# pbluc/avrecode-ms

Measured on AMD Instinct MI355X. Metric: H.264 bytes/s recompressed (CABAC re-encode of recorded bin streams, bit-exact vs CPU), higher is better.
Workload: dtype u32

## Files before the change

avrecode-ms_amd/csrc/avr_api.cpp:

```cpp
#include <hip/hip_runtime.h>

#include <algorithm>
#include <cstdarg>
#include <cstdio>
#include <cstdlib>
#include <cstring>
#include <mutex>
#include <new>
#include <numeric>
#include <string>
#include <thread>
#include <vector>

#include "avr_internal.h"
#include "avr_synth.h"
#include "avr_tables.h"

namespace {

thread_local char g_err[512] = "";

int fail(int code, const char *fmt, ...) {
    va_list ap;
    va_start(ap, fmt);
// ... 125 lines not shown
    avr_chunk_plan plan{};

    bool verify = false;
    bool verified = false;
    hipEvent_t vev[3] = {};
    float verify_ms = 0;
    DevBuf<uint32_t> d_first_bad;
    PinBuf<uint32_t> h_first_bad;
};

template <class T>
static int stage_h2d(avr_batch *b, T *dst, const T *src, size_t n) {
    const size_t bytes = n * sizeof(T), at = (b->plan_used + 63) & ~size_t(63);
    if (at + bytes > b->h_plan.cap) return fail(AVR_ERR_NOMEM, "plan staging area too small (%zu + %zu > %zu)", at, bytes, b->h_plan.cap);
    memcpy(b->h_plan.p + at, src, bytes);
    b->plan_used = at + bytes;
    AVR_HIP(hipMemcpyAsync(dst, b->h_plan.p + at, bytes, hipMemcpyHostToDevice, b->stream));
    return AVR_OK;
}
namespace avr {
const Env &env() {
    static const Env e = [] {
        Env v{0, false, false};
        if (const char *p = getenv("AVR_K1_PATH")) v.k1_path = strcmp(p, "chunked") == 0 ? 2 : strcmp(p, "serial") == 0 ? 1 : 0;
        v.no_dense = getenv("AVR_NO_DENSE") != nullptr;
        v.no_hint = getenv("AVR_BATCH_NO_HINT") != nullptr;
        return v;
    }();
    return e;
}
#ifdef AVR_TEST_HOOKS
TestHooks &test_hooks() { static TestHooks h{}; return h; }
#endif
}

extern "C" {

#ifdef AVR_TEST_HOOKS
int avr_test_hook_set(const char *name, uint32_t value) {
    avr::TestHooks &h = avr::test_hooks();
    if (!name) return fail(AVR_ERR_INVALID, "null hook name");
    if (!strcmp(name, "k1p_force_retry_every")) h.k1p_force_retry_every = value;
    else if (!strcmp(name, "census_stride")) h.census_stride = value;
    else if (!strcmp(name, "chain_lanes")) h.chain_lanes = value;
    else if (!strcmp(name, "k1_form_ref")) h.k1_form_ref = value;
    else if (!strcmp(name, "k1_emit_lds")) h.k1_emit_lds = value;
    else if (!strcmp(name, "k1_path")) h.k1_path = value;
    else if (!strcmp(name, "no_dense")) h.no_dense = value;
    else if (!strcmp(name, "no_hint")) h.no_hint = value;
    else if (!strcmp(name, "k2p_seg_len")) h.k2p_seg_len = value;
    else if (!strcmp(name, "local_waves")) h.local_waves = value;
    else if (!strcmp(name, "k2p_wave")) h.k2p_wave = value;
    else if (!strcmp(name, "k1p_keep_retry")) h.k1p_keep_retry = value;
    else if (!strcmp(name, "k1_waves")) h.k1_waves = value;
    else if (!strcmp(name, "k1_fwd")) h.k1_fwd = value;
    else if (!strcmp(name, "k1_words8")) h.k1_words8 = value;
    else if (!strcmp(name, "chain_nsegs")) h.chain_nsegs = value;
    else if (!strcmp(name, "chain_whole")) h.chain_whole = value;
    else if (!strcmp(name, "chain_segments")) h.chain_segments = value;
    else if (!strcmp(name, "chain_force_redo")) h.chain_force_redo = value;
    else if (!strcmp(name, "verify_flip")) h.verify_flip = value;
    else if (!strcmp(name, "reset")) h = avr::TestHooks{};
    else return fail(AVR_ERR_INVALID, "unknown test hook %s", name);
    return AVR_OK;
}
#endif

const char *avr_last_error(void) { return g_err; }
const char *avr_version(void) { return "avrecode-ms_amd 0.1 (gfx950)"; }

int avr_device_count(void) {
    int n = 0;
    if (hipGetDeviceCount(&n) != hipSuccess) return 0;
    return n;
}

const uint8_t *avr_cabac_lps_range_table(void) { return kTables.lps_range; }
const uint8_t *avr_cabac_mlps_state_table(void) { return kTables.mlps_state; }


avr_batch *avr_batch_create(int device, size_t max_slices, size_t max_bins) {
    if (max_slices == 0 || max_slices > 0x7fffffffu) { fail(AVR_ERR_INVALID, "max_slices out of range"); return nullptr; }
    if (select_device(device) != AVR_OK) return nullptr;
    avr_batch *b = new (std::nothrow) avr_batch;
    if (!b) { fail(AVR_ERR_NOMEM, "out of host memory"); return nullptr; }
    b->device = device;
    b->max_slices = max_slices;
    b->max_bins = max_bins;
    bool ok = hipStreamCreateWithFlags(&b->stream, hipStreamNonBlocking) == hipSuccess;
    for (int i = 0; ok && i < 5; i++) ok = hipEventCreate(&b->ev[i]) == hipSuccess;
    ok = ok && b->h_recs.reserve(max_bins + 16 * max_slices) == AVR_OK;
    if (!ok) {
        if (!g_err[0]) fail(AVR_ERR_HIP, "stream/event creation failed");
        avr_batch_destroy(b);
        return nullptr;
    }
    b->rec_off.reserve(max_slices + 1);
    b->n_bins.reserve(max_slices);
    b->rec_off.push_back(0);
    return b;
}

void avr_batch_destroy(avr_batch *b) {
    if (!b) return;
    (void)hipSetDevice(b->device);
    if (b->stream) (void)hipStreamSynchronize(b->stream);
// ... 1217 lines not shown
```

avrecode-ms_amd/csrc/avr_internal.h:

```cpp
#pragma once
#include <hip/hip_runtime.h>
#include <stdint.h>

#include <list>
#include <mutex>

#include "../../include/avrecode_ms_amd.h"
#include "avr_layout.h"

#define AVR_NOP_CABAC2  (AVR_NOP_CABAC | (AVR_NOP_CABAC << 16))
#define AVR_SLICE_RETRY_SERIAL 100
#define AVR_SLICE_RETRY_CENSUS 101
#define AVR_SLICE_DONE         102

namespace avr {

struct Env { int k1_path; bool no_dense, no_hint; };
const Env &env();
struct TestHooks {
    uint32_t k1p_force_retry_every;
    uint32_t census_stride;
    uint32_t chain_lanes;
    uint32_t k1_form_ref;
    uint32_t k1_emit_lds;
    uint32_t k1_path, no_dense, no_hint;
    uint32_t chain_segments;
    uint32_t chain_whole;
    uint32_t chain_force_redo;
    uint32_t k2p_seg_len;
    uint32_t local_waves;
    uint32_t chain_nsegs;
    uint32_t k1_fwd;
    uint32_t k1_words8;
    uint32_t k1_waves;
    uint32_t k2p_wave;
    uint32_t verify_flip;
    uint32_t k1p_keep_retry;
};
#ifdef AVR_TEST_HOOKS
TestHooks &test_hooks();
#else
inline const TestHooks &test_hooks() { static const TestHooks none{}; return none; }
#endif
inline int k1_path() { return test_hooks().k1_path ? int(test_hooks().k1_path) : env().k1_path; }
inline bool no_dense() { return test_hooks().no_dense || env().no_dense; }
inline bool no_hint() { return test_hooks().no_hint || env().no_hint; }

struct DenseHint { uint32_t rows; uint32_t *host_count; uint32_t *host_retry; uint32_t sharing = 0; };

template <class T>
class StreamPool {
    struct Slot { int dev; hipStream_t s; T x; };
    std::list<Slot> slots_;
    std::mutex mu_;
public:
    template <class Make>
    hipError_t get(hipStream_t s, T **out, Make make) {
        int dev = 0;
        hipError_t e = hipGetDevice(&dev);
        if (e != hipSuccess) return e;
        std::lock_guard<std::mutex> lock(mu_);
        for (Slot &x : slots_)
            if (x.dev == dev && x.s == s) { *out = &x.x; return hipSuccess; }
        T fresh{};
        if ((e = make(fresh)) != hipSuccess) return e;
        slots_.push_back(Slot{dev, s, fresh});
        *out = &slots_.back().x;
        return hipSuccess;
    }
    template <class Destroy>
    void forget(hipStream_t s, Destroy destroy) {
        std::lock_guard<std::mutex> lock(mu_);
        for (auto it = slots_.begin(); it != slots_.end();)
            if (it->s == s) { destroy(it->x); it = slots_.erase(it); } else ++it;
    }
};

void forget_stream(hipStream_t s);
void forget_part_streams(hipStream_t s);

hipError_t launch_cabac_encode(bool tiled, hipStream_t s, const void *recs, const uint64_t *off,
                               const uint32_t *n_bins, const uint32_t *order, uint32_t n_slices,
                               const uint8_t *init_states, uint32_t n_states, uint8_t *out,
                               const uint64_t *out_off, uint32_t *out_len, int32_t *status,
                               uint8_t *final_states, int32_t want_status = AVR_SLICE_OK, bool dense = true,
                               const DenseHint *hint = nullptr);
hipError_t launch_densemap(hipStream_t s, const uint32_t *used, uint16_t *table, uint16_t *index, uint32_t *n_dense);
hipError_t launch_range_encode(bool tiled, hipStream_t s, const void *recs, const uint64_t *off,
                               const uint32_t *n_bins, const uint32_t *order, uint32_t n_slices,
                               uint8_t *out, const uint64_t *out_off, uint32_t *out_len,
// ... 60 lines not shown
```

avrecode-ms_amd/csrc/avr_k1p.h:

```cpp
#pragma once
#include <stdint.h>

#if defined(__HIPCC__)
#define AVR_HD __host__ __device__ inline
#else
#define AVR_HD inline
#endif

namespace avr {
namespace k1p {

#if defined(__HIP_DEVICE_COMPILE__)
#define AVR_PIN2(a, b) asm volatile("" : "+v"(a), "+v"(b))
#else
#define AVR_PIN2(a, b) ((void)0)
#endif

constexpr uint32_t kChunk = 1024;
constexpr uint32_t kNone = 0xffffffffu;
constexpr uint32_t kMaxStretch = 16 * kChunk;
constexpr uint32_t kCodeBypass = 252;
constexpr uint32_t kCodePad = 252;

struct alignas(16) U4 { uint32_t x, y, z, w; };
// ... 196 lines not shown
            const U4 v = *reinterpret_cast<const U4 *>(res + i);
            const uint32_t w[4] = {v.x, v.y, v.z, v.w};
#if defined(__HIP_DEVICE_COMPILE__)
#pragma unroll 1
#endif
            for (uint32_t k = 0; k < 4; k++) {
                CodeEntry e[4];
                code_entries4(codes, w[k], e);
                for (uint32_t b = 0; b < 4; b++)
                    for (uint32_t q = 0; q < 4; q++) T[q] += step_range(e[b], &R[q]);
            }
            i += 16;
        }
        code_by_code(n);
    }
    uint32_t Rm = R[0], Tm = 0, end = i;
    if (!closed && i < n) {
        const uint32_t interior_end = limit < n ? limit : n;
        if (i < interior_end) {
            for_codes_all(res, i, interior_end, [&](uint32_t c) { Tm += step_range(codes[c], &Rm); },
                          [&](uint32_t d) {
                              CodeEntry e[4];
                              code_entries4(codes, d, e);
                              Tm += step_range(e[0], &Rm); Tm += step_range(e[1], &Rm);
                              Tm += step_range(e[2], &Rm); Tm += step_range(e[3], &Rm);
                          });
            i = interior_end;
        }
        end = n;
        for_codes(res, i, n, [&](uint32_t idx, uint32_t c) {
            const bool closing = idx >= limit && code_is_boundary(c);
            if (closing) o->exit_q = uint8_t(((Rm >> 6) & 3) * 0x55u);
            Tm += step_range(codes[c], &Rm);
            if (closing) { end = idx + 1; return true; }
            if (idx - lo > max_stretch) { o->too_long = 1; end = idx + 1; return true; }
            return false;
        });
        R[0] = R[1] = R[2] = R[3] = Rm;
    }
    o->end = end;
    for (uint32_t q = 0; q < 4; q++) { o->t_exit[q] = T[q] + Tm; o->r_exit[q] = uint16_t(R[q]); }
}


struct Entry {
    uint32_t t_start;
    uint32_t q;
};

struct SliceTotals {
    uint32_t t_total;
    uint32_t r_final;
    uint32_t bad;
    uint32_t pad;
};

AVR_HD void b2_chain(const Stretch *st, uint32_t n_chunks, Entry *en, SliceTotals *tot) {
    uint32_t T = 0, q = 0, r = 510, bad = 0;
    for (uint32_t c = 0; c < n_chunks; c++) {
        if (st[c].first == kNone) continue;
        en[c].t_start = T;
        en[c].q = q;
        T += st[c].t_exit[q];
        r = st[c].r_exit[q];
        bad |= st[c].too_long;
        q = (st[c].exit_q >> (2 * q)) & 3;
    }
    tot->t_total = T;
    tot->r_final = r;
    tot->bad = bad;
    tot->pad = 0;
}

AVR_HD uint32_t ref_digits(uint32_t t) { return t <= 21 ? 0 : (t - 21 + 15) / 16; }


template <class A, class = void> struct adder_is_staged { static constexpr bool value = false; };
template <class A> struct adder_is_staged<A, decltype(void(A::kStaged))> { static constexpr bool value = A::kStaged; };
template <class Src, class Adder>
AVR_HD void c_stretch_in(const Src &src, const Stretch &st, const Entry &en, uint32_t chunk,
                         const CodeEntryC *codes, Adder &S) {
    uint32_t R, from;
    if (chunk == 0) { R = 510; from = 0; }
    else { uint32_t sh; R = post_lps_range(codes[src.byte(st.first)].row, en.q, &sh); from = st.first + 1; }
    const uint32_t phase = en.t_start & 15, g0 = en.t_start >> 4;
    uint64_t L2 = 0;
    int sp = int(phase) - 7;
    uint32_t j = 0;
    constexpr bool staged = adder_is_staged<Adder>::value;
    if constexpr (staged) S.begin(g0);
    auto bin_e = [&](const CodeEntryC &e) {
        uint32_t v;
        const uint32_t sh = step_range_c(e, &R, &v);
        L2 = (L2 + v) << sh;
        sp += int(sh);
    };
    auto bin = [&](uint32_t c) { bin_e(codes[c]); };
    auto put = [&](uint32_t d) {
        if constexpr (staged) S.push(g0 + j, d);
        else if (j < 2) S.add(g0 + j, d);
        else S.store(g0 + j, d);
        j++;
    };
    auto digits = [&]() {
        while (sp >= 15) {
            const uint32_t d = uint32_t(L2 >> (sp + 1));
            L2 &= (uint64_t(2) << sp) - 1;
            put(d);
            sp -= 16;
        }
    };
    auto digits2 = [&]() {
        const int s1 = sp + 1;
        const uint32_t nd = uint32_t(s1 > 0 ? s1 : 0) >> 4, ks = 16 + (uint32_t(s1) & 15u);
        const uint64_t t = L2 >> ks;
        const uint32_t a = nd == 2 ? uint32_t(t >> 16) : uint32_t(t), b = uint32_t(t) & 0xffffu;
        L2 = uint32_t(L2) & (nd ? (1u << ks) - 1 : ~0u);
        sp -= int(16 * nd);
        if constexpr (staged) { S.push2(nd, a, b); j += nd; S.look(g0 + j); }
        else { if (nd) put(a); if (nd == 2) put(b); }
    };
    const uint32_t to = st.end;
    if (from < to) {
        auto four = [&](uint32_t d) {
            CodeEntryC e[4];
            code_entries4(codes, d, e);
            bin_e(e[0]); bin_e(e[1]); bin_e(e[2]); bin_e(e[3]);
            digits2();
        };
        auto group16 = [&](const U4 &v) { four(v.x); four(v.y); four(v.z); four(v.w); };
        const uint32_t head_end = ((from + 15) & ~15u) < to ? ((from + 15) & ~15u) : to;
        for_codes_in(src, from, head_end, [&](uint32_t, uint32_t c) { bin(c); digits(); return false; });
        uint32_t base = head_end;
        for (; (base & 63) && base + 16 <= to; base += 16) group16(src.load16(base));
        U4 v0{0, 0, 0, 0}, v1 = v0, v2 = v0, v3 = v0;
        if (base + 64 <= to) { v0 = src.load16(base); v1 = src.load16(base + 16); v2 = src.load16(base + 32); v3 = src.load16(base + 48); }
        for (; base + 64 <= to; base += 64) {
            const uint32_t w[16] = {v0.x, v0.y, v0.z, v0.w, v1.x, v1.y, v1.z, v1.w, v2.x, v2.y, v2.z, v2.w, v3.x, v3.y, v3.z, v3.w};
            const uint32_t nb = base + 128 <= to ? base + 64 : base;
            v0 = src.load16(nb); v1 = src.load16(nb + 16); v2 = src.load16(nb + 32); v3 = src.load16(nb + 48);
#if defined(__HIP_DEVICE_COMPILE__)
#pragma unroll 4
#endif
            for (uint32_t k = 0; k < 16; k++) four(w[k]);
        }
        for (; base + 16 <= to; base += 16) group16(src.load16(base));
        if (base < to) for_codes_in(src, base, to, [&](uint32_t, uint32_t c) { bin(c); digits(); return false; });
    }
    if constexpr (staged) S.flush(g0 + j);
    else S.flush();
    if (sp >= 0) {
        S.add(g0 + j, uint32_t(L2 >> (sp + 1)));
        S.add(g0 + j + 1, uint32_t(L2 & ((uint64_t(2) << sp) - 1)) << (15 - sp));
    } else {
        S.add(g0 + j, uint32_t(L2 << (-sp - 1)) );
    }
}

template <class Adder>
AVR_HD void c_stretch(const uint8_t *res, const Stretch &st, const Entry &en, uint32_t chunk,
                      const CodeEntryC *codes, Adder &S) {
    c_stretch_in(LinearCodes{res}, st, en, chunk, codes, S);
}


AVR_HD uint32_t d_finish(uint32_t low, uint32_t range, uint8_t tail[5], uint32_t *carry) {
    for (uint32_t stop = 1u << 30; stop > 0; stop >>= 1) {
        const uint32_t x = (low | stop) & ~(stop - 1);
        if (stop < range && low <= x && x < uint32_t(low + range)) { low = x; break; }
    }
    uint32_t n = 0, cy = 0;
    while (low != 0 && n < 5) {
        if (low >= 0x80000000u) { cy = 1; low -= 0x80000000u; }
        const uint32_t d = low >> 23;
        tail[n++] = uint8_t(d);
        low = (low - (d << 23)) << 8;
    }
    *carry = cy;
    return n;
}

AVR_HD uint32_t d_slice(const uint32_t *S, const SliceTotals &tot, uint8_t *out, uint32_t cap) {
    const uint32_t nd = ref_digits(tot.t_total);
    const uint32_t low = uint32_t((uint64_t(S[nd]) << 15) + (S[nd + 1] >> 1));
    const uint32_t range = tot.r_final << (22 - tot.t_total + 16 * nd);
    uint8_t tail[5];
    uint32_t carry;
    const uint32_t n_tail = d_finish(low, range, tail, &carry);
    for (uint32_t i = nd; i-- > 0;) {
        const uint32_t v = S[i] + carry;
        carry = v >> 16;
        if (2 * i + 1 < cap) { out[2 * i] = uint8_t(v >> 8); out[2 * i + 1] = uint8_t(v); }
    }
    for (uint32_t k = 0; k < n_tail; k++)
        if (2 * nd + k < cap) out[2 * nd + k] = tail[k];
    return 2 * nd + n_tail;
}

}
}
```

avrecode-ms_amd/csrc/avr_k1p.hip:

```cpp
#include <hip/hip_runtime.h>

#include <mutex>
#include <stdint.h>
#include <stdlib.h>
#include <type_traits>

#include "avr_coder.h"
#include "avr_internal.h"
#include "avr_k1p.h"
#include "avr_tables.h"

namespace avr {

static __device__ const CabacTables d_tables = make_cabac_tables();

using namespace k1p;

constexpr uint32_t kSortBlock = AVR_SORT_BLOCK_BINS;

struct Plan {
    const uint16_t *recs;
    const uint64_t *rec_off;
    const uint32_t *n_bins;
    const uint64_t *res_off;
// ... 863 lines not shown
    if (gc >= total_chunks) return;
    const uint32_t slice = p.chunk_slice[gc];
    if (status[slice] != AVR_SLICE_OK) { st[gc].first = kNone; st[gc].too_long = 0; return; }
    const uint32_t c = gc - p.chunk_base[slice], n = p.n_bins[slice], i0 = c * kChunk;
    const uint32_t i1 = i0 + kChunk < n ? i0 + kChunk : n;
    const uint8_t *r = res + p.res_off[slice];
    B1Walk b1;
    b1.init(c, i0, i1, n, max_stretch, codes2);
    auto eight = [&](uint32_t lo, uint32_t hi, uint4 e[8]) {
#pragma unroll
        for (uint32_t j = 0; j < 8; j++) e[j] = cinfo[((j < 4 ? lo : hi) >> (8 * (j & 3))) & 0xffu];
    };
    uint8_t *to = tile ? tile + ((size_t(gc >> 6) * 64) * 64 + (gc & 63u)) * 16 : nullptr;
    auto sixteen = [&](uint32_t base, const U4 &v) {
        if (to) *reinterpret_cast<U4 *>(to + size_t((base - i0) >> 4) * 1024) = v;
        uint4 e[8];
        eight(v.x, v.y, e); b1.group(base, e);
        eight(v.z, v.w, e); b1.group(base + 8, e);
    };
    uint32_t i = i0;
    if (i0 < n) {
        U4 v0{0, 0, 0, 0}, v1 = v0, v2 = v0, v3 = v0;
        if (i + 64 <= i1) { const U4 *q = reinterpret_cast<const U4 *>(r + i); v0 = q[0]; v1 = q[1]; v2 = q[2]; v3 = q[3]; }
        for (; i + 64 <= i1; i += 64) {
            const U4 *qn = reinterpret_cast<const U4 *>(r + (i + 128 <= i1 ? i + 64 : i));
            const U4 n0 = qn[0], n1 = qn[1], n2 = qn[2], n3 = qn[3];
            sixteen(i, v0); sixteen(i + 16, v1); sixteen(i + 32, v2); sixteen(i + 48, v3);
            v0 = n0; v1 = n1; v2 = n2; v3 = n3;
        }
        for (; i < i1; i += 16) sixteen(i, *reinterpret_cast<const U4 *>(r + i));
        b1.chunk_done();
        for (i = i0 + kChunk; b1.mode != 3 && i < n; i += 16) {
            const U4 v = *reinterpret_cast<const U4 *>(r + i);
            uint4 e[8];
            eight(v.x, v.y, e); b1.tail(i, e);
            if (b1.mode != 3) { eight(v.z, v.w, e); b1.tail(i + 8, e); }
        }
    }
    st[gc] = b1.finish();
}

constexpr uint32_t kB2Tile = 1024, kB2Seg = 16;

__global__ __launch_bounds__(256) void k_k1p_b2(Plan p, const int32_t *status, const Stretch *st, Entry *en,
                                                SliceTotals *tot, uint32_t *S) {
    __shared__ Stretch tile[kB2Tile];
    __shared__ Entry ent[kB2Tile];
    __shared__ uint8_t xq[kB2Tile], qin[kB2Tile];
    __shared__ uint8_t segmap[256], segin[kB2Tile / kB2Seg];
    __shared__ uint32_t wsum[4];
    __shared__ uint32_t carry[4];
    const uint32_t s = blockIdx.x, t = threadIdx.x, lane = t & 63, w = t >> 6;
    if (status[s] != AVR_SLICE_OK) {
        if (t == 0) { tot[s].t_total = 0; tot[s].r_final = 510; tot[s].bad = 0; tot[s].pad = 0; }
        return;
    }
    const uint32_t c0 = p.chunk_base[s], nc = p.chunk_base[s + 1] - c0;
    if (t == 0) { carry[0] = 0; carry[1] = 0; carry[2] = 510; carry[3] = 0; }
    for (uint32_t base = 0; base < nc; base += kB2Tile) {
        const uint32_t cnt = nc - base < kB2Tile ? nc - base : kB2Tile;
        const uint32_t *src = reinterpret_cast<const uint32_t *>(st + c0 + base);
        uint32_t *dst = reinterpret_cast<uint32_t *>(tile);
        for (uint32_t i = t; i < cnt * (sizeof(Stretch) / 4); i += 256) dst[i] = src[i];
        __syncthreads();
        for (uint32_t c = t; c < kB2Tile; c += 256) xq[c] = c < cnt && tile[c].first != kNone ? tile[c].exit_q : uint8_t(0xE4);
        __syncthreads();
        {
            const uint32_t seg = t >> 2, c_lo = seg * kB2Seg;
            uint32_t q = t & 3u;
            for (uint32_t c = c_lo; c < c_lo + kB2Seg; c++) q = (xq[c] >> (2 * q)) & 3;
            segmap[t] = uint8_t(q);
        }
        __syncthreads();
        if (t == 0) {
            uint32_t q = carry[1];
            for (uint32_t sg = 0; sg < kB2Tile / kB2Seg; sg++) { segin[sg] = uint8_t(q); q = segmap[4 * sg + q]; }
            carry[1] = q;
        }
        __syncthreads();
        if (t < kB2Tile / kB2Seg) {
            uint32_t q = segin[t];
            for (uint32_t c = t * kB2Seg; c < (t + 1) * kB2Seg; c++) { qin[c] = uint8_t(q); q = (xq[c] >> (2 * q)) & 3; }
        }
        __syncthreads();
        uint32_t tv[4], sum = 0, bad = 0, last = kNone;
#pragma unroll
        for (uint32_t j = 0; j < 4; j++) {
            const uint32_t c = 4 * t + j;
            const bool on = c < cnt && tile[c].first != kNone;
            tv[j] = on ? tile[c].t_exit[qin[c]] : 0;
            sum += tv[j];
            if (on) { bad |= tile[c].too_long; last = c; }
        }
        uint32_t incl = sum;
        for (uint32_t d = 1; d < 64; d <<= 1) { const uint32_t v = __shfl_up(incl, d); if (lane >= d) incl += v; }
        if (lane == 63) wsum[w] = incl;
        const uint64_t has = __ballot(last != kNone);
        __syncthreads();
        uint32_t run = carry[0] + incl - sum;
        for (uint32_t v = 0; v < w; v++) run += wsum[v];
#pragma unroll
        for (uint32_t j = 0; j < 4; j++) {
            const uint32_t c = 4 * t + j;
            if (c < cnt) { ent[c].t_start = run; ent[c].q = qin[c]; }
            run += tv[j];
        }
        if (bad) atomicOr(&carry[3], 1u);
        __syncthreads();
        if (t == 255) carry[0] = run;
        for (uint32_t v = 0; v < 4; v++) {
            if (w == v && has && lane == 63 - uint32_t(__builtin_clzll(has))) carry[2] = tile[last].r_exit[qin[last]];
            __syncthreads();
        }
        uint32_t *eo = reinterpret_cast<uint32_t *>(en + c0 + base);
        const uint32_t *ei = reinterpret_cast<const uint32_t *>(ent);
        for (uint32_t i = t; i < cnt * (sizeof(Entry) / 4); i += 256) eo[i] = ei[i];
        __syncthreads();
    }
    if (t == 0) { tot[s].t_total = carry[0]; tot[s].r_final = carry[2]; tot[s].bad = carry[3]; tot[s].pad = 0; }
    __syncthreads();
    const uint32_t n = ref_digits(carry[0]) + 2;
    uint32_t *d = S + p.dig_off[s];
    for (uint32_t i = t; i < n; i += 256) d[i] = 0;
}

constexpr uint32_t kRing = 16, kFull = kRing - 2;
struct DeviceAdder {
    static constexpr bool kStaged = true;
    uint32_t *S;
    uint32_t *ring;
    uint32_t g0 = 0, cnt = 0;
    __device__ __forceinline__ void begin(uint32_t g) { g0 = g; }
    __device__ __forceinline__ void push2(uint32_t nd, uint32_t a, uint32_t b) {
        ring[cnt * 64] = a;
        ring[cnt * 64 + 64] = b;
        cnt += nd;
    }
    __device__ __forceinline__ void look(uint32_t i) { if (__ballot(cnt >= kFull) != 0) drain(i, false); }
    __device__ __forceinline__ void push(uint32_t i, uint32_t v) {
        if (cnt >= kFull) drain(i, false);
        ring[cnt * 64] = v;
        cnt++;
    }
    __device__ __forceinline__ void flush(uint32_t i) { drain(i, true); }
    typedef __attribute__((address_space(1))) uint32_t GlobalWord;
    typedef __attribute__((address_space(3))) uint32_t LdsWord;
    __device__ __forceinline__ void drain(uint32_t i, bool last) { cnt = drain_staged((GlobalWord *)S, (LdsWord *)ring, g0, cnt, i, last); }
    static __device__ __noinline__ uint32_t drain_staged(GlobalWord *S, LdsWord *ring, uint32_t g0, uint32_t cnt, uint32_t i, bool last) {
        const uint32_t first = i - cnt, word = uint32_t(reinterpret_cast<uintptr_t>(S) >> 2) + first;
        uint32_t k = 0;
#pragma unroll 1
        while (k < cnt) {
            const uint32_t a = (word + k) & 3u, left = cnt - k;
            LdsWord *r = ring + k * 64;
            if (first + k < g0 + 2) { atomicAdd((uint32_t *)&S[first + k], r[0]); k++; }
            else if (a == 0 && left >= 4) { *(uint4 *)(S + first + k) = make_uint4(r[0], r[64], r[128], r[192]); k += 4; }
            else if (last || (a != 0 && left >= 4 - a)) { S[first + k] = r[0]; k++; }
            else break;
        }
        cnt -= k;
        if (k != 0) {
#pragma unroll 1
            for (uint32_t m = 0; m < cnt; m++) ring[m * 64] = ring[(k + m) * 64];
        }
        return cnt;
    }
    __device__ void add(uint32_t i, uint32_t v) { atomicAdd(&S[i], v); }
};

template <bool TILE_CODES>
__global__ __launch_bounds__(256, 7) void k_k1p_c(Plan p, uint32_t total_chunks, const uint8_t *res,
                                                  const Stretch *st, const Entry *en, const SliceTotals *tot,
                                                  uint32_t *S) {
    __shared__ CodeEntryC codes[256];
    __shared__ uint32_t ring[kRing * 256];
    codes[threadIdx.x] = code_entry_c(device_code_entry(threadIdx.x));
    __syncthreads();
    const uint32_t gc = blockIdx.x * 256 + threadIdx.x;
    if (gc >= total_chunks) return;
    const Stretch o = st[gc];
    if (o.first == kNone) return;
    const uint32_t slice = p.chunk_slice[gc];
    if (tot[slice].bad) return;
    DeviceAdder add;
    add.S = S + p.dig_off[slice];
    add.ring = ring + (threadIdx.x >> 6) * (kRing * 64) + (threadIdx.x & 63u);
    if (TILE_CODES) c_stretch_in(TileCodes{res, p.chunk_base[slice]}, o, en[gc], gc - p.chunk_base[slice], codes, add);
    else c_stretch(res + p.res_off[slice], o, en[gc], gc - p.chunk_base[slice], codes, add);
}


constexpr uint32_t kSeg = 33;
constexpr uint32_t kTile = 256 * kSeg;

__global__ __launch_bounds__(256) void k_k1p_d(Plan p, const SliceTotals *tot, const uint32_t *S,
                                               uint8_t *out, const uint64_t *out_off, uint32_t *out_len,
                                               int32_t *status, uint32_t force_retry_every) {
    __shared__ uint32_t dig[kTile];
    __shared__ uint32_t seg_g[256], seg_cin[256];
    __shared__ uint64_t seg_gm[4], seg_pm[4];
    __shared__ uint32_t sh_carry;
    const uint32_t s = blockIdx.x, t = threadIdx.x;
    if (status[s] != AVR_SLICE_OK) { if (t == 0 && status[s] != AVR_SLICE_DONE) out_len[s] = 0; return; }
    const SliceTotals T = tot[s];
    if (T.bad || (force_retry_every && s % force_retry_every == 0)) { if (t == 0) status[s] = AVR_SLICE_RETRY_SERIAL; return; }
    const uint32_t *Ss = S + p.dig_off[s];
    uint8_t *o = out + out_off[s];
    const uint32_t cap = uint32_t(out_off[s + 1] - out_off[s]);
    const uint32_t nd = ref_digits(T.t_total);
    if (t == 0) {
        const uint32_t low = uint32_t((uint64_t(Ss[nd]) << 15) + (Ss[nd + 1] >> 1));
        const uint32_t range = T.r_final << (22 - T.t_total + 16 * nd);
        uint8_t tail[5];
        uint32_t carry;
        const uint32_t n_tail = d_finish(low, range, tail, &carry);
        for (uint32_t k = 0; k < n_tail; k++) {
            if (2 * nd + k < cap) o[2 * nd + k] = tail[k];
        }
        sh_carry = carry;
        out_len[s] = 2 * nd + n_tail;
        if (2 * nd + n_tail > cap) status[s] = AVR_SLICE_OVERFLOW;
    }
    __syncthreads();
    uint32_t carry_in = sh_carry;
    for (uint32_t hi = nd; hi > 0;) {
        const uint32_t lo = hi > kTile ? hi - kTile : 0, cnt = hi - lo;
        for (uint32_t i = t; i < cnt; i += 256) dig[i] = Ss[lo + i];
        __syncthreads();
        const uint32_t a = t * kSeg < cnt ? t * kSeg : cnt, b = (t + 1) * kSeg < cnt ? (t + 1) * kSeg : cnt;
        uint32_t c = 0, all_ones = 1;
        for (uint32_t i = b; i-- > a;) {
            const uint32_t v = dig[i] + c;
            dig[i] = v & 0xffffu;
            c = v >> 16;
            all_ones &= (v & 0xffffu) == 0xffffu;
        }
        const bool gen = c > 0, prop = all_ones && !gen;
        const uint64_t gm = __builtin_bitreverse64(__ballot(gen)), pm = __builtin_bitreverse64(__ballot(prop));
        if ((t & 63) == 0) { seg_gm[t >> 6] = gm; seg_pm[t >> 6] = pm; }
        __syncthreads();
        uint32_t into = carry_in > 0;
        bool recv = false;
        for (uint32_t v = 4; v-- > 0;) {
            const uint64_t a = seg_gm[v] | seg_pm[v], b2 = seg_gm[v], sum = a + b2 + into;
            if (v == (t >> 6)) recv = (__builtin_bitreverse64(sum ^ a ^ b2) >> (t & 63)) & 1;
            into = uint32_t(((a & b2) | ((a | b2) & ~sum)) >> 63);
        }
        seg_g[t] = c + ((all_ones && recv) ? 1u : 0u);
        __syncthreads();
        const uint32_t n_seg = (cnt + kSeg - 1) / kSeg;
        seg_cin[t] = t + 1 >= n_seg ? carry_in : seg_g[t + 1];
        if (t == 0) sh_carry = seg_g[0];
        __syncthreads();
        if (t < n_seg && seg_cin[t]) {
            uint32_t c2 = seg_cin[t];
            for (uint32_t i = b; i-- > a && c2;) {
                const uint32_t v = dig[i] + c2;
                dig[i] = v & 0xffffu;
                c2 = v >> 16;
            }
            if (c2 != ((all_ones && recv) ? 1u : 0u)) status[s] = AVR_SLICE_RETRY_SERIAL;
        }
        __syncthreads();
        for (uint32_t i = t; i < cnt; i += 256) {
            const uint32_t v = dig[i], at = 2 * (lo + i);
            if (at + 1 < cap) *reinterpret_cast<uint16_t *>(o + at) = uint16_t((v >> 8) | (v << 8));
        }
        carry_in = sh_carry;
        hi = lo;
        __syncthreads();
    }
}

template <bool TILE>
__global__ __launch_bounds__(64) void k_cabac_encode_codes(const uint8_t *codes_in, const uint64_t *res_off, const uint32_t *chunk_base,
                                                           const uint32_t *n_bins, const uint32_t *order, uint32_t n_slices, uint8_t *out,
                                                           const uint64_t *out_off, uint32_t *out_len, int32_t *status,
                                                           int32_t want_status) {
    __shared__ CodeEntry codes[256];
    for (uint32_t c = threadIdx.x; c < 256; c += 64) codes[c] = device_code_entry(c);
    __syncthreads();
    const uint32_t g = blockIdx.x * 64 + threadIdx.x;
    if (g >= n_slices) return;
    const uint32_t slice = order ? order[g] : g;
    if (status[slice] != want_status) {
        if (want_status == AVR_SLICE_OK) out_len[slice] = 0;
        return;
    }
    const uint32_t n = n_bins[slice];
    const uint8_t *res = TILE ? codes_in : codes_in + res_off[slice];
    const TileCodes tiled{codes_in, TILE ? chunk_base[slice] : 0u};
    auto load16 = [&](uint32_t i) { return TILE ? tiled.load16(i) : *reinterpret_cast<const U4 *>(res + i); };
    auto byte = [&](uint32_t i) { return TILE ? tiled.byte(i) : uint32_t(res[i]); };
    const uint64_t o0 = out_off[slice];
    const uint32_t cap = uint32_t(out_off[slice + 1] - o0);
    CabacEncoder e;
    e.init(0x7F800000u, out + o0, cap);
    auto bin = [&](uint32_t c) {
        const CodeEntry ce = codes[c];
        const int norm = 23 - __builtin_clz(e.range);
        const uint32_t q = (e.range >> (norm + 6)) & 3;
        const uint32_t r_tab = ((ce.row >> (8 * q)) & 0xffu) << norm;
        const uint32_t r1 = (ce.meta >> 8) ? e.range >> 1 : r_tab;
        const uint32_t sym = (ce.meta >> 1) & 1u;
        const uint32_t r0 = e.range - r1;
        e.low += sym ? r0 : 0u;
        e.range = sym ? r1 : r0;
        if (e.range < 0x200u) e.emit_digit();
    };
    uint32_t i = 0;
    if (n >= 16) {
        U4 v = load16(0);
        for (; i + 16 <= n; i += 16) {
            const U4 nx = i + 32 <= n ? load16(i + 16) : v;
// ... 125 lines not shown
                                    : hipSuccess;
            }
            if (e != hipSuccess) return e;
        }
        hipLaunchKernelGGL(local, dim3((pl->total_chunks + 64 * waves - 1) / (64 * waves)), dim3(64 * waves), lds, s, p,
                           pl->total_chunks, status, lbits, lend, n_retry);
        if (mode.census_stride > 1 && !mode.second_pass) {
            if (hint && hint->rows && hint->host_retry) {
                if ((e = hipMemcpyAsync(hint->host_retry, n_retry, 4, hipMemcpyDeviceToHost, s)) != hipSuccess) return e;
            } else if (mode.retry_count) {
                if ((e = hipMemcpyAsync(mode.retry_count, n_retry, 4, hipMemcpyDeviceToHost, s)) != hipSuccess) return e;
                if ((e = hipStreamSynchronize(s)) != hipSuccess) return e;
            }
        }
    }
    if (n_states > 0) {
        uint32_t chain_lanes = uint32_t((uint64_t(n_slices) * n_states + 2047) / 2048);
        chain_lanes = chain_lanes < kChainLanes ? kChainLanes : chain_lanes > 64 ? 64 : chain_lanes;
        if (const uint32_t v = test_hooks().chain_lanes) chain_lanes = v <= 64 ? v : 64;
        const bool packed = chain_lanes == 64;
        const uint32_t groups = packed ? 0u : (n_states + chain_lanes - 1) / chain_lanes;
        const uint32_t whole_waves = packed ? uint32_t((uint64_t(n_slices) * n_states + 63) / 64) : n_slices * groups;
        const dim3 whole((whole_waves + kChainWaves - 1) / kChainWaves), block(64 * kChainWaves);
        const bool few_lanes = uint64_t(n_slices) * n_states <= 49152;
        const uint32_t pair_waves = uint32_t((uint64_t(n_slices) * n_states + 63) / 64);
        uint32_t n_segs = kChainWaveSlots / (pair_waves * (hint && hint->sharing ? hint->sharing : 1u));
        n_segs = n_segs > kMaxChainSegs ? kMaxChainSegs : n_segs;
        const uint64_t by_length = uint64_t(pl->total_chunks) / (uint64_t(n_slices) * 4);
        if (n_segs > by_length) n_segs = uint32_t(by_length);
        if (const uint32_t v = test_hooks().chain_nsegs) n_segs = v < kMaxChainSegs ? v : kMaxChainSegs;
        if (n_segs >= 2 && !test_hooks().chain_whole && (few_lanes || test_hooks().chain_segments)) {
            SegSummary *summ = reinterpret_cast<SegSummary *>(w + L.summ);
            const dim3 seg_grid((pair_waves * n_segs + kSegWaves - 1) / kSegWaves), seg_block(64 * kSegWaves);
            hipLaunchKernelGGL(k_k1p_chain_seg, seg_grid, seg_block, 0, s, p, n_slices, n_segs, status, tn, lbits, lend, est, summ);
            hipLaunchKernelGGL(k_k1p_chain_fix, seg_grid, seg_block, 0, s, p, n_slices, n_segs, status, tn, lbits, lend, init_states, est, summ,
                               final_states, test_hooks().chain_force_redo);
        } else {
            hipLaunchKernelGGL(k_k1p_ctxchain, whole, block, 0, s, p, n_slices, groups, chain_lanes, status, tn, lbits, lend, init_states, est, final_states);
        }
    }
    const uint32_t per_wave = ((n_states + 8) / 4) * 256;
    const uint32_t replay_waves = per_wave * 4 <= 48 * 1024 ? 4 : per_wave * 2 <= 48 * 1024 ? 2 : 1;
    const uint32_t replay_lds = replay_waves * per_wave;
    auto replay = r8 ? k_k1p_replay<true, true> : mode.tile_codes ? k_k1p_replay<true, false> : k_k1p_replay<false, false>;
    if (replay_lds > 48 * 1024) {
        e = hipFuncSetAttribute(reinterpret_cast<const void *>(replay), hipFuncAttributeMaxDynamicSharedMemorySize, int(replay_lds));
        if (e != hipSuccess) return e;
    }
    hipLaunchKernelGGL(replay, dim3((pl->total_chunks + 64 * replay_waves - 1) / (64 * replay_waves)), dim3(64 * replay_waves),
                       replay_lds, s, p, pl->total_chunks, reinterpret_cast<const uint32_t *>(est), res, status, stretch, max_stretch);
    return hipGetLastError();
}

static hipError_t launch_code(hipStream_t s, const Plan &p, uint32_t n_slices, const avr_chunk_plan *pl, uint8_t *w,
                              const uint8_t *res, uint32_t max_stretch, const K1pIo &io, const Stretch *have = nullptr,
                              bool tile_codes = false) {
    const CodeLayout L = code_layout(n_slices, pl);
    Stretch *st_own = reinterpret_cast<Stretch *>(w + L.stretch);
    const Stretch *st = have ? have : st_own;
    Entry *en = reinterpret_cast<Entry *>(w + L.entry);
    SliceTotals *tot = reinterpret_cast<SliceTotals *>(w + L.totals);
    uint32_t *S = reinterpret_cast<uint32_t *>(w + L.sums);
    const uint32_t chunk_blocks = (pl->total_chunks + 255) / 256;
    if (!have) {
        uint8_t *tile = w + L.tile;
        hipLaunchKernelGGL(k_k1p_b1, dim3(chunk_blocks), dim3(256), 0, s, p, pl->total_chunks, res, io.status, st_own, max_stretch, tile);
        res = tile;
        tile_codes = true;
    }
    hipLaunchKernelGGL(k_k1p_b2, dim3(n_slices), dim3(256), 0, s, p, io.status, st, en, tot, S);
    if (tile_codes) hipLaunchKernelGGL(k_k1p_c<true>, dim3(chunk_blocks), dim3(256), 0, s, p, pl->total_chunks, res, st, en, tot, S);
    else hipLaunchKernelGGL(k_k1p_c<false>, dim3(chunk_blocks), dim3(256), 0, s, p, pl->total_chunks, res, st, en, tot, S);
    const uint32_t force_retry_every = test_hooks().k1p_force_retry_every;
    hipLaunchKernelGGL(k_k1p_d, dim3(n_slices), dim3(256), 0, s, p, tot, S, io.out, io.out_off, io.out_len, io.status, force_retry_every);
    return hipGetLastError();
}

hipError_t launch_densemap(hipStream_t s, const uint32_t *used, uint16_t *table, uint16_t *index, uint32_t *n_dense) {
    hipLaunchKernelGGL(k_k1p_densemap, dim3(1), dim3(1024), 0, s, used, table, index, n_dense);
    return hipGetLastError();
}

hipError_t launch_cabac_encode_codes(hipStream_t s, const uint8_t *codes, const uint64_t *res_off, const uint32_t *n_bins,
                                     const uint32_t *order, uint32_t n_slices, uint8_t *out, const uint64_t *out_off,
                                     uint32_t *out_len, int32_t *status, int32_t want_status) {
    if (n_slices == 0) return hipSuccess;
    hipLaunchKernelGGL(k_cabac_encode_codes<false>, dim3((n_slices + 63) / 64), dim3(64), 0, s, codes, res_off, nullptr, n_bins, order,
                       n_slices, out, out_off, out_len, status, want_status);
    return hipGetLastError();
}

constexpr uint32_t kK1pCensusStride = 16;

static uint32_t census_stride() {
    return test_hooks().census_stride ? test_hooks().census_stride : kK1pCensusStride;
}

struct K1pJob { Plan p; uint32_t n_slices; const avr_chunk_plan *pl; uint8_t *codes, *resolve_ws, *code_ws; };
static K1pJob k1p_job(Records kind, const void *recs, const uint64_t *rec_off, const uint32_t *n_bins, uint32_t n_slices,
                      uint32_t n_states, const avr_chunk_plan *pl, void *workspace) {
    const K1pLayout L = k1p_layout(n_slices, n_states, pl);
    uint8_t *w = static_cast<uint8_t *>(workspace);
    return K1pJob{make_plan(kind, recs, rec_off, n_bins, n_states, pl), n_slices, pl, w + L.codes, w + L.resolve, w + L.code};
}

static hipError_t k1p_stages(hipStream_t s, const K1pJob &j, const K1pIo &io, ResolveMode mode) {
    const Stretch *st = nullptr;
    mode.tile_codes = true;
    hipError_t e = launch_resolve(s, j.p, j.n_slices, j.pl, j.resolve_ws, j.codes, io, kMaxStretch, &st, mode);
    if (e != hipSuccess) return e;
    return launch_code(s, j.p, j.n_slices, j.pl, j.code_ws, j.codes, kMaxStretch, io, st, true);
}

static hipError_t k1p_pass(hipStream_t s, const K1pJob &j, const K1pIo &io, const ResolveMode &mode) {
    const hipError_t e = k1p_stages(s, j, io, mode);
    if (e != hipSuccess || test_hooks().k1p_keep_retry) return e;
    return launch_cabac_encode(false, s, j.p.recs, j.p.rec_off, j.p.n_bins, nullptr, j.n_slices, io.init_states, j.p.ns_full, io.out,
                               io.out_off, io.out_len, io.status, nullptr, AVR_SLICE_RETRY_SERIAL);
}

template <class Pass>
static hipError_t k1p_second_pass(hipStream_t s, uint32_t n_slices, int32_t *status, Pass pass) {
    const dim3 grid((n_slices + 255) / 256), block(256);
    hipLaunchKernelGGL(k_k1p_swap, grid, block, 0, s, status, n_slices, AVR_SLICE_OK, AVR_SLICE_DONE, AVR_SLICE_RETRY_CENSUS, AVR_SLICE_OK);
    ResolveMode mode;
    mode.second_pass = true;
    const hipError_t e = pass(mode);
// ... 69 lines not shown
```

Before: 24.99 billion.

## Split digit carry-propagation kernel into multiple pieces per slice

The final carry-resolve kernel k_k1p_d now launches a 2D grid with several workgroups per slice. Each non-last piece finds its incoming carry by scanning forward for a digit that cannot propagate a carry, using a wave ballot, and falls back to the tail computation if none is found. The b2 kernel also stops zero-filling the whole digit array and only zeroes the digit slots each chunk will touch, plus the two trailing ones. This is meant to raise parallelism on long slices when slice count is low, at the cost of redundant carry scans and atomic status updates.

Result: no change. 25.19 billion, median of 6 (+0.8%).

```diff
diff --git a/avrecode-ms_amd/csrc/avr_api.cpp b/avrecode-ms_amd/csrc/avr_api.cpp
--- a/avrecode-ms_amd/csrc/avr_api.cpp
+++ b/avrecode-ms_amd/csrc/avr_api.cpp
@@ -201,6 +201,7 @@
     else if (!strcmp(name, "local_waves")) h.local_waves = value;
     else if (!strcmp(name, "k2p_wave")) h.k2p_wave = value;
     else if (!strcmp(name, "k1p_keep_retry")) h.k1p_keep_retry = value;
+    else if (!strcmp(name, "d_pieces")) h.d_pieces = value;
     else if (!strcmp(name, "k1_waves")) h.k1_waves = value;
     else if (!strcmp(name, "k1_fwd")) h.k1_fwd = value;
     else if (!strcmp(name, "k1_words8")) h.k1_words8 = value;
diff --git a/avrecode-ms_amd/csrc/avr_internal.h b/avrecode-ms_amd/csrc/avr_internal.h
--- a/avrecode-ms_amd/csrc/avr_internal.h
+++ b/avrecode-ms_amd/csrc/avr_internal.h
@@ -36,6 +36,7 @@
     uint32_t k2p_wave;
     uint32_t verify_flip;
     uint32_t k1p_keep_retry;
+    uint32_t d_pieces;
 };
 #ifdef AVR_TEST_HOOKS
 TestHooks &test_hooks();
diff --git a/avrecode-ms_amd/csrc/avr_k1p.h b/avrecode-ms_amd/csrc/avr_k1p.h
--- a/avrecode-ms_amd/csrc/avr_k1p.h
+++ b/avrecode-ms_amd/csrc/avr_k1p.h
@@ -272,7 +272,7 @@
     uint32_t t_total;
     uint32_t r_final;
     uint32_t bad;
-    uint32_t pad;
+    uint32_t skip;
 };
 
 AVR_HD void b2_chain(const Stretch *st, uint32_t n_chunks, Entry *en, SliceTotals *tot) {
@@ -289,7 +289,7 @@
     tot->t_total = T;
     tot->r_final = r;
     tot->bad = bad;
-    tot->pad = 0;
+    tot->skip = 0;
 }
 
 AVR_HD uint32_t ref_digits(uint32_t t) { return t <= 21 ? 0 : (t - 21 + 15) / 16; }
@@ -383,6 +383,16 @@
     c_stretch_in(LinearCodes{res}, st, en, chunk, codes, S);
 }
 
+AVR_HD void c_shared_digits(uint32_t t_start, uint32_t t_shifts, uint32_t at[4]) {
+    const uint32_t g0 = t_start >> 4;
+    const int64_t s1 = int64_t(t_start & 15) - 6 + int64_t(t_shifts);
+    const uint32_t j = s1 > 0 ? uint32_t(s1 >> 4) : 0;
+    at[0] = g0;
+    at[1] = g0 + (j ? 1u : 0u);
+    at[2] = g0 + j;
+    at[3] = g0 + j + (s1 - 16 * int64_t(j) >= 1 ? 1u : 0u);
+}
+
 
 AVR_HD uint32_t d_finish(uint32_t low, uint32_t range, uint8_t tail[5], uint32_t *carry) {
     for (uint32_t stop = 1u << 30; stop > 0; stop >>= 1) {
@@ -400,10 +410,16 @@
     return n;
 }
 
+AVR_HD void d_window(const uint32_t *S, const SliceTotals &tot, uint32_t *low, uint32_t *range) {
+    const uint32_t nd = ref_digits(tot.t_total);
+    *low = uint32_t((uint64_t(S[nd]) << 15) + (S[nd + 1] >> 1));
+    *range = tot.r_final << (22 - tot.t_total + 16 * nd);
+}
+
 AVR_HD uint32_t d_slice(const uint32_t *S, const SliceTotals &tot, uint8_t *out, uint32_t cap) {
     const uint32_t nd = ref_digits(tot.t_total);
-    const uint32_t low = uint32_t((uint64_t(S[nd]) << 15) + (S[nd + 1] >> 1));
-    const uint32_t range = tot.r_final << (22 - tot.t_total + 16 * nd);
+    uint32_t low, range;
+    d_window(S, tot, &low, &range);
     uint8_t tail[5];
     uint32_t carry;
     const uint32_t n_tail = d_finish(low, range, tail, &carry);
@@ -417,5 +433,62 @@
     return 2 * nd + n_tail;
 }
 
-}
-}
+constexpr uint32_t kMaxPieces = 64;
+AVR_HD uint32_t d_piece_begin(uint32_t nd, uint32_t piece, uint32_t n_pieces) { return uint32_t(uint64_t(nd) * piece / n_pieces); }
+
+constexpr uint32_t kCarryMax = 256;
+AVR_HD uint32_t ctz64(uint64_t x) { return uint32_t(__builtin_ctzll(x)); }
+template <class Wave>
+AVR_HD uint32_t d_carry_into(const uint32_t *S, const SliceTotals &tot, uint32_t from, const Wave &wave) {
+    const uint32_t nd = ref_digits(tot.t_total);
+    uint32_t m = from, c = 0;
+    bool decided = false;
+    for (; m < nd; m += 64) {
+        const uint64_t mask = wave.ballot([&](uint32_t lane) { return m + lane < nd && (S[m + lane] & 0xffffu) + kCarryMax < 0x10000u; });
+        if (mask) { m += ctz64(mask); c = S[m] >> 16; decided = true; break; }
+    }
+    if (!decided) {
+        uint32_t low, range;
+        uint8_t tail[5];
+        d_window(S, tot, &low, &range);
+        d_finish(low, range, tail, &c);
+        m = nd;
+    }
+    for (uint32_t i = m; i-- > from;) c = (S[i] + c) >> 16;
+    return c;
+}
+struct SerialWave {
+    template <class F> uint64_t ballot(F &&f) const {
+        uint64_t mask = 0;
+        for (uint32_t lane = 0; lane < 64; lane++) mask |= uint64_t(f(lane) ? 1 : 0) << lane;
+        return mask;
+    }
+};
+
+AVR_HD uint32_t d_piece(const uint32_t *S, const SliceTotals &tot, uint32_t piece, uint32_t n_pieces, uint8_t *out, uint32_t cap) {
+    const uint32_t nd = ref_digits(tot.t_total);
+    const uint32_t lo = d_piece_begin(nd, piece, n_pieces), hi = d_piece_begin(nd, piece + 1, n_pieces);
+    const bool last = piece + 1 == n_pieces;
+    uint32_t carry, len = 0;
+    if (last) {
+        uint32_t low, range;
+        uint8_t tail[5];
+        d_window(S, tot, &low, &range);
+        const uint32_t n_tail = d_finish(low, range, tail, &carry);
+        for (uint32_t k = 0; k < n_tail; k++)
+            if (2 * nd + k < cap) out[2 * nd + k] = tail[k];
+        len = 2 * nd + n_tail;
+    } else {
+        if (lo == hi) return 0;
+        carry = d_carry_into(S, tot, hi, SerialWave{});
+    }
+    for (uint32_t i = hi; i-- > lo;) {
+        const uint32_t v = S[i] + carry;
+        carry = v >> 16;
+        if (2 * i + 1 < cap) { out[2 * i] = uint8_t(v >> 8); out[2 * i + 1] = uint8_t(v); }
+    }
+    return len;
+}
+
+}
+}
diff --git a/avrecode-ms_amd/csrc/avr_k1p.hip b/avrecode-ms_amd/csrc/avr_k1p.hip
--- a/avrecode-ms_amd/csrc/avr_k1p.hip
+++ b/avrecode-ms_amd/csrc/avr_k1p.hip
@@ -939,10 +939,11 @@
     __shared__ uint32_t carry[4];
     const uint32_t s = blockIdx.x, t = threadIdx.x, lane = t & 63, w = t >> 6;
     if (status[s] != AVR_SLICE_OK) {
-        if (t == 0) { tot[s].t_total = 0; tot[s].r_final = 510; tot[s].bad = 0; tot[s].pad = 0; }
+        if (t == 0) { tot[s].t_total = 0; tot[s].r_final = 510; tot[s].bad = 0; tot[s].skip = 1; }
         return;
     }
     const uint32_t c0 = p.chunk_base[s], nc = p.chunk_base[s + 1] - c0;
+    uint32_t *d = S + p.dig_off[s];
     if (t == 0) { carry[0] = 0; carry[1] = 0; carry[2] = 510; carry[3] = 0; }
     for (uint32_t base = 0; base < nc; base += kB2Tile) {
         const uint32_t cnt = nc - base < kB2Tile ? nc - base : kB2Tile;
@@ -990,6 +991,11 @@
         for (uint32_t j = 0; j < 4; j++) {
             const uint32_t c = 4 * t + j;
             if (c < cnt) { ent[c].t_start = run; ent[c].q = qin[c]; }
+            if (c < cnt && tile[c].first != kNone) {
+                uint32_t at[4];
+                c_shared_digits(run, tv[j], at);
+                d[at[0]] = 0; d[at[1]] = 0; d[at[2]] = 0; d[at[3]] = 0;
+            }
             run += tv[j];
         }
         if (bad) atomicOr(&carry[3], 1u);
@@ -1004,11 +1010,11 @@
         for (uint32_t i = t; i < cnt * (sizeof(Entry) / 4); i += 256) eo[i] = ei[i];
         __syncthreads();
     }
-    if (t == 0) { tot[s].t_total = carry[0]; tot[s].r_final = carry[2]; tot[s].bad = carry[3]; tot[s].pad = 0; }
-    __syncthreads();
-    const uint32_t n = ref_digits(carry[0]) + 2;
-    uint32_t *d = S + p.dig_off[s];
-    for (uint32_t i = t; i < n; i += 256) d[i] = 0;
+    if (t == 0) {
+        tot[s].t_total = carry[0]; tot[s].r_final = carry[2]; tot[s].bad = carry[3]; tot[s].skip = 0;
+        const uint32_t nd = ref_digits(carry[0]);
+        d[nd] = 0; d[nd + 1] = 0;
+    }
 }
 
 constexpr uint32_t kRing = 16, kFull = kRing - 2;
@@ -1080,6 +1086,10 @@
 constexpr uint32_t kSeg = 33;
 constexpr uint32_t kTile = 256 * kSeg;
 
+struct DeviceWave {
+    template <class F> __device__ __forceinline__ uint64_t ballot(F &&f) const { return __ballot(f(threadIdx.x & 63u)); }
+};
+
 __global__ __launch_bounds__(256) void k_k1p_d(Plan p, const SliceTotals *tot, const uint32_t *S,
                                                uint8_t *out, const uint64_t *out_off, uint32_t *out_len,
                                                int32_t *status, uint32_t force_retry_every) {
@@ -1087,31 +1097,41 @@
     __shared__ uint32_t seg_g[256], seg_cin[256];
     __shared__ uint64_t seg_gm[4], seg_pm[4];
     __shared__ uint32_t sh_carry;
-    const uint32_t s = blockIdx.x, t = threadIdx.x;
-    if (status[s] != AVR_SLICE_OK) { if (t == 0 && status[s] != AVR_SLICE_DONE) out_len[s] = 0; return; }
+    const uint32_t s = blockIdx.x, t = threadIdx.x, piece = blockIdx.y, n_pieces = gridDim.y;
+    const bool last_piece = piece + 1 == n_pieces;
     const SliceTotals T = tot[s];
-    if (T.bad || (force_retry_every && s % force_retry_every == 0)) { if (t == 0) status[s] = AVR_SLICE_RETRY_SERIAL; return; }
+    if (T.skip) { if (last_piece && t == 0 && status[s] != AVR_SLICE_DONE) out_len[s] = 0; return; }
+    if (T.bad || (force_retry_every && s % force_retry_every == 0)) { if (last_piece && t == 0) status[s] = AVR_SLICE_RETRY_SERIAL; return; }
     const uint32_t *Ss = S + p.dig_off[s];
     uint8_t *o = out + out_off[s];
     const uint32_t cap = uint32_t(out_off[s + 1] - out_off[s]);
     const uint32_t nd = ref_digits(T.t_total);
-    if (t == 0) {
-        const uint32_t low = uint32_t((uint64_t(Ss[nd]) << 15) + (Ss[nd + 1] >> 1));
-        const uint32_t range = T.r_final << (22 - T.t_total + 16 * nd);
-        uint8_t tail[5];
-        uint32_t carry;
-        const uint32_t n_tail = d_finish(low, range, tail, &carry);
-        for (uint32_t k = 0; k < n_tail; k++) {
-            if (2 * nd + k < cap) o[2 * nd + k] = tail[k];
-        }
-        sh_carry = carry;
-        out_len[s] = 2 * nd + n_tail;
-        if (2 * nd + n_tail > cap) status[s] = AVR_SLICE_OVERFLOW;
+    const uint32_t p_lo = d_piece_begin(nd, piece, n_pieces), p_hi = d_piece_begin(nd, piece + 1, n_pieces);
+    if (last_piece) {
+        if (t == 0) {
+            uint32_t low, range;
+            d_window(Ss, T, &low, &range);
+            uint8_t tail[5];
+            uint32_t carry;
+            const uint32_t n_tail = d_finish(low, range, tail, &carry);
+            for (uint32_t k = 0; k < n_tail; k++) {
+                if (2 * nd + k < cap) o[2 * nd + k] = tail[k];
+            }
+            sh_carry = carry;
+            out_len[s] = 2 * nd + n_tail;
+            if (2 * nd + n_tail > cap) atomicMax(&status[s], int32_t(AVR_SLICE_OVERFLOW));
+        }
+    } else {
+        if (p_lo == p_hi) return;
+        if (t < 64) {
+            const uint32_t carry = d_carry_into(Ss, T, p_hi, DeviceWave{});
+            if (t == 0) sh_carry = carry;
+        }
     }
     __syncthreads();
     uint32_t carry_in = sh_carry;
-    for (uint32_t hi = nd; hi > 0;) {
-        const uint32_t lo = hi > kTile ? hi - kTile : 0, cnt = hi - lo;
+    for (uint32_t hi = p_hi; hi > p_lo;) {
+        const uint32_t lo = hi - p_lo > kTile ? hi - kTile : p_lo, cnt = hi - lo;
         for (uint32_t i = t; i < cnt; i += 256) dig[i] = Ss[lo + i];
         __syncthreads();
         const uint32_t a = t * kSeg < cnt ? t * kSeg : cnt, b = (t + 1) * kSeg < cnt ? (t + 1) * kSeg : cnt;
@@ -1146,7 +1166,7 @@
                 dig[i] = v & 0xffffu;
                 c2 = v >> 16;
             }
-            if (c2 != ((all_ones && recv) ? 1u : 0u)) status[s] = AVR_SLICE_RETRY_SERIAL;
+            if (c2 != ((all_ones && recv) ? 1u : 0u)) atomicMax(&status[s], int32_t(AVR_SLICE_RETRY_SERIAL));
         }
         __syncthreads();
         for (uint32_t i = t; i < cnt; i += 256) {
@@ -1378,6 +1398,14 @@
     return hipGetLastError();
 }
 
+constexpr uint32_t kDWorkgroups = 2048, kDPieceChunks = 32, kDPieces = 8;
+static uint32_t d_pieces(uint32_t n_slices, uint32_t total_chunks) {
+    if (const uint32_t v = test_hooks().d_pieces) return v < kMaxPieces ? v : kMaxPieces;
+    const uint32_t by_count = kDWorkgroups / n_slices, by_length = total_chunks / n_slices / kDPieceChunks;
+    const uint32_t n = by_count < by_length ? by_count : by_length;
+    return n < 1 ? 1 : n > kDPieces ? kDPieces : n;
+}
+
 static hipError_t launch_code(hipStream_t s, const Plan &p, uint32_t n_slices, const avr_chunk_plan *pl, uint8_t *w,
                               const uint8_t *res, uint32_t max_stretch, const K1pIo &io, const Stretch *have = nullptr,
                               bool tile_codes = false) {
@@ -1398,7 +1426,8 @@
     if (tile_codes) hipLaunchKernelGGL(k_k1p_c<true>, dim3(chunk_blocks), dim3(256), 0, s, p, pl->total_chunks, res, st, en, tot, S);
     else hipLaunchKernelGGL(k_k1p_c<false>, dim3(chunk_blocks), dim3(256), 0, s, p, pl->total_chunks, res, st, en, tot, S);
     const uint32_t force_retry_every = test_hooks().k1p_force_retry_every;
-    hipLaunchKernelGGL(k_k1p_d, dim3(n_slices), dim3(256), 0, s, p, tot, S, io.out, io.out_off, io.out_len, io.status, force_retry_every);
+    hipLaunchKernelGGL(k_k1p_d, dim3(n_slices, d_pieces(n_slices, pl->total_chunks)), dim3(256), 0, s, p, tot, S, io.out, io.out_off, io.out_len,
+                       io.status, force_retry_every);
     return hipGetLastError();
 }
 
```
